# broadinstitute/colab-repeat-finder

Measured on AMD Instinct MI355X. Metric: Gbp/s scanned (motif 1-50), higher is better.
Workload: dtype u32 bit planes (2-bit bases)

## Files before the change

### colab-repeat-finder_amd/csrc/prf_plan.h

```cpp
#pragma once
#include <stdint.h>

typedef unsigned long long u64;
typedef unsigned int u32;

#define PRF_VMAX_K 480
#define PRF_VMAX_TASKS 80
#define PRF_VMAX_WAVES 4
#define PRF_GATHER_SLOTS_MAX 64u
#define PRF_GATHER_SUPER 64u
#define PRF_LAUNCH_MIXED 0x80000000u

struct alignas(4) prf_vtask {
    unsigned short k0;
    unsigned char kind;
    unsigned char valid;
    unsigned char stride;
    unsigned char pad;
    unsigned short item0;
};

struct prf_vplan {
    u32 n_waves;
    u32 n_tasks;
    u32 wave_begin[PRF_VMAX_WAVES + 1];
    prf_vtask tasks[PRF_VMAX_TASKS];
    u32 nc;
    u32 lds_bytes;
    u32 cof_words;
    u32 n_group_k;
    u32 n_exact;
    u32 k_exact0;
    u32 ticket_wave;
    u32 slack_waves;
    u32 per_cu;
    u32 prio;
};


namespace prf_layout {
constexpr int T = 32;
constexpr int RG = T / 4;
constexpr int LIN_PRE = 2;
constexpr int LIN_POST = 24;
constexpr int TILE_WORDS = 1024;
constexpr int LW = TILE_WORDS + LIN_PRE + LIN_POST;
constexpr int REC_CAP = 192;
constexpr int FLAG_CAP = 960;
constexpr int SLOW_CAP = 16;
constexpr int SMALL_M = 15;
constexpr int ROW_CAP_LDS = 448;
constexpr int SMEM_HDR = 240;
}

static inline long long prf_plan_min_matches(u32 k, u32 min_repeats, u32 min_span) {
    const long long a = (long long)(min_repeats - 1) * (long long)k, b = (long long)min_span - (long long)k;
    return a > b ? a : b;
}

bool prf_vertical_plan(u32 kmin, u32 kmax, u32 min_repeats, u32 min_span, prf_vplan *plan);
int prf_plan_json(u32 kmin, u32 kmax, u32 min_repeats, u32 min_span, char *buf, u64 buf_len);
```

### colab-repeat-finder_amd/csrc/scan_host.cpp

```cpp
#include <hip/hip_runtime.h>

#include <algorithm>
#include <chrono>
#include <cstdio>
#include <cstdlib>
#include <cstring>
#include <vector>

#include "genome.h"

template <class T>
static int grow(T *&p, u64 &cap, u64 want) {
    if (want <= cap) return PRF_OK;
    (void)hipFree(p);
    p = nullptr;
    cap = 0;
    HIPCHK(hipMalloc((void **)&p, want * sizeof(T)));
    cap = want;
    return PRF_OK;
}

static u64 with_headroom(u64 n) { return n + n / 8 + 1024; }

extern "C" {
// ... 91 lines not shown
    c->slab_slots = nslots;
    c->slab_cap = cap;
    return PRF_OK;
}

static int launch_fused(prf_ctx *c, const prf_genome *g, const prf_vplan &plan, const scan_params &p, prf_hit_dev *rows, u64 rows_cap,
                        u32 count_row, u64 *host_counters_dev, u64 *seq_out) {
    const launch_view lv = active_launch(g);
    prf_vscan_args a;
    a.VH = g->vp.VH; a.VL = g->vp.VL;
    a.H = g->H; a.L = g->L; a.X = g->X;
    a.E = g->d_E;
    a.launch_list = lv.list; a.n_launch = lv.n; a.flat_base = lv.flat;
    a.slabs = c->d_slabs; a.long_ends = c->d_long_ends; a.slab_count = c->d_slab_count; a.block_sum = c->d_block_sum; a.slab_cap = c->slab_cap;
    a.gather_shift = lv.n <= 8192u ? 3u : 5u;
#ifdef PRF_DIAG
    {
        static const int gs_env = getenv("PRF_GATHER_SHIFT") ? atoi(getenv("PRF_GATHER_SHIFT")) : -1;
        if (gs_env >= 3 && gs_env <= 6) a.gather_shift = (u32)gs_env;
    }
    {
        static const u32 skip_env = getenv("PRF_SKIP") ? (u32)strtoul(getenv("PRF_SKIP"), nullptr, 0) : 0u;
        a.skip = skip_env;
    }
#endif
    a.super_off = (lv.n + (1u << a.gather_shift) - 1u) >> a.gather_shift;
    a.min_repeats = p.min_repeats; a.min_span = p.min_span;
    a.tile_info = g->d_tile_info;
    a.counters = c->d_vcounters + (size_t)c->parity * PRF_CNT_N;
    a.dbg = nullptr;
#ifdef PRF_STAMPS
    {
        static u64 *dbg_buf = nullptr;
        const size_t nu = (size_t)(1u << 18) * PRF_VMAX_WAVES * 16;
        if (!dbg_buf) HIPCHK(hipMalloc((void **)&dbg_buf, nu * sizeof(u64)));
        if (lv.n <= (1u << 18)) {
            HIPCHK(hipMemsetAsync(dbg_buf, 0, (size_t)lv.n * PRF_VMAX_WAVES * 16 * sizeof(u64), c->stream));
            a.dbg = dbg_buf;
            c->stamps_buf = dbg_buf;
            c->stamps_n = lv.n;
        }
    }
#endif
    a.plan = plan;
    prf_vgather_args ga;
    ga.slabs = c->d_slabs; ga.long_ends = c->d_long_ends; ga.launch_list = lv.list; ga.flat_base = lv.flat; ga.tile_info = g->d_tile_info;
    ga.slab_count = c->d_slab_count; ga.block_sum = c->d_block_sum; ga.slab_cap = c->slab_cap; ga.n_launch = lv.n;
    ga.super_off = a.super_off;
    ga.gather_shift = a.gather_shift;
    ga.rows = rows; ga.rows_cap = rows_cap; ga.count_row = count_row;
    ga.counters = a.counters;
    ga.host_counters = host_counters_dev;
    ga.seq = ++c->scan_seq;
    ga.next_counters = c->d_vcounters + (size_t)(c->parity ^ 1u) * PRF_CNT_N;
    c->parity ^= 1u;
    const hipEvent_t *ev = ring_events(c, ga.seq);
    HIPCHK(hipEventRecord(ev[0], c->stream));
    hipError_t le = prf_vertical_launch(c->stream, a);
    if (le == hipSuccess) le = hipEventRecord(ev[1], c->stream);
    if (le == hipSuccess) le = prf_vertical_gather(c->stream, ga);
    if (le != hipSuccess) {
        reset_vcounters(c);
        return fail(PRF_EHIP, "fused scan launch failed: %s", hipGetErrorString(le));
    }
    HIPCHK(hipEventRecord(ev[2], c->stream));
    *seq_out = ga.seq;
    return PRF_OK;
}

struct row_dest {
// ... 35 lines not shown
    r.sorted = h[PRF_CNT_UNSORTED] == 0;
    r.ncand = shard_sum(h, PRF_SH_CAND);
    r.launches = 2;
    return r;
}

static void fill_stats(prf_scan_stats *s, const pass_result &r, u32 path, u64 positions, u32 tiles, u64 seq) {
    memset(s, 0, sizeof *s);
    s->phase1_ms = r.ms01;
    s->phase2_ms = r.ms12;
    s->scan_ms = (double)r.ms01 + (double)r.ms12;
    s->positions = positions;
    s->packed_bytes = (positions + 3) / 4;
    s->n_candidates = r.ncand;
    s->n_hits = r.nhits;
    s->n_launches = r.launches;
    s->path = path;
    s->seq = seq;
    s->sorted_on_device = r.sorted ? 1u : 0u;
    s->tiles_launched = tiles;
}

#ifdef PRF_STAMPS
static int dump_stamps(prf_ctx *c, const prf_vplan &plan) {
    const char *path = getenv("PRF_STAMPS_OUT");
    if (!path) return PRF_OK;
    fprintf(stderr, "[prf] plan: %u waves, %u tasks\n", plan.n_waves, plan.n_tasks);
    for (u32 w = 0; w < plan.n_waves; w++)
        for (u32 ti = plan.wave_begin[w]; ti < plan.wave_begin[w + 1]; ti++)
            fprintf(stderr, "[prf]   wave %u slot %u: kind %u k0 %u valid %02x stride %u\n", w, ti - plan.wave_begin[w],
                    plan.tasks[ti].kind, plan.tasks[ti].k0, plan.tasks[ti].valid, plan.tasks[ti].stride);
    if (c->stamps_buf) {
        HIPCHK(hipStreamSynchronize(c->stream));
        const size_t nu = (size_t)c->stamps_n * PRF_VMAX_WAVES * 16;
        std::vector<u64> host(nu);
        HIPCHK(hipMemcpy(host.data(), c->stamps_buf, nu * sizeof(u64), hipMemcpyDeviceToHost));
        if (FILE *f = fopen(path, "wb")) { fwrite(host.data(), 8, nu, f); fclose(f); }
    }
    return PRF_OK;
}
#endif

static int fused_pass(prf_ctx *c, const prf_genome *g, const prf_vplan &plan, const scan_params &p, const row_dest &dst, bool timed,
                      buffer_sizes *want, pass_result *r) {
    u64 seq = 0;
    int rc = launch_fused(c, g, plan, p, dst.rows, dst.cap, dst.is_sink ? 1u : 0u, c->h_counters_dev, &seq);
    if (rc) return rc;
    rc = wait_for_seq(c, seq);
    if (rc) return rc;
#ifdef PRF_STAMPS
    rc = dump_stamps(c, plan);
    if (rc) return rc;
#endif
    if (dst.is_sink) HIPCHK(hipStreamSynchronize(c->stream));
    const u64 *h = c->h_counters;
    *r = read_fused(h);
    if (timed) {
        const hipEvent_t *ev = ring_events(c, seq);
        HIPCHK(hipEventSynchronize(ev[2]));
        HIPCHK(hipEventElapsedTime(&r->ms01, ev[0], ev[2]));
    }
#ifdef PRF_DIAG
    if (getenv("PRF_DEBUG"))
        fprintf(stderr, "[prf] fused: hits %llu cand-records %llu (verified on the spot, a list being full: %llu) hit_ovf %llu unsorted %llu ms %.4f\n",
                (unsigned long long)r->nhits, (unsigned long long)r->ncand, (unsigned long long)shard_sum(h, PRF_SH_EARLY),
                (unsigned long long)h[PRF_CNT_HIT_OVF], (unsigned long long)h[PRF_CNT_UNSORTED], r->ms01);
#endif
// ... 275 lines not shown
```

### colab-repeat-finder_amd/csrc/scan_vertical.h

```cpp
#pragma once
#include <hip/hip_runtime.h>

#include <vector>

#include "prf_device.h"

#include "prf_plan.h"

struct prf_vplanes {
    u32 *VH = nullptr, *VL = nullptr;
    unsigned char *tile_class = nullptr;
    u32 *launch_list = nullptr;
    u32 n_launch = 0;
    u32 flat_base = ~0u;
    u64 ntiles_alloc = 0;
    std::vector<unsigned char> h_class;
    std::vector<u32> h_list;
};

#define PRF_LONG_PER_TILE 4u

struct prf_vscan_args {
    const u32 *VH, *VL;
    const u64 *H, *L, *X;
    const u64 *const *E;
    const u32 *launch_list;
    u32 n_launch;
    u32 flat_base;
    u64 *slabs;
    u64 *long_ends;
    u32 *slab_count;
    u32 *block_sum;
    u32 super_off;
    u32 gather_shift;
    u32 slab_cap;
    u32 min_repeats, min_span;
    const uint4 *tile_info;
    u64 *counters;
    u64 *dbg;
#ifdef PRF_DIAG
    u32 skip;
#endif
    prf_vplan plan;
};

struct prf_vgather_args {
    const u64 *slabs;
    const u64 *long_ends;
    const u32 *slab_count;
    const u32 *launch_list;
    u32 flat_base;
    const uint4 *tile_info;
    u32 *block_sum;
// ... 22 lines not shown
```

### colab-repeat-finder_amd/csrc/scan_vertical.hip

```cpp
#include <algorithm>
#include <cstdio>
#include <cstdlib>
#include <utility>
#include <vector>

#include "prf_host.h"
#include "prf_static_for.h"
#include "scan_vertical.h"
#include "verify_impl.h"

namespace {

#include "vscan_common.h"
#include "vscan_verify.h"
#include "vscan_tasks.h"

__device__ __forceinline__ void set_prio(u32 p) {
#ifdef PRF_NO_PRIO
    return;
#endif
    if (p == 0u) __builtin_amdgcn_s_setprio(0);
    else if (p == 1u) __builtin_amdgcn_s_setprio(1);
    else if (p == 2u) __builtin_amdgcn_s_setprio(2);
    else __builtin_amdgcn_s_setprio(3);
// ... 114 lines not shown
        tcw->slab_cap = g.slab_cap;
        tcw->min_repeats = g.min_repeats;
        tcw->min_span = g.min_span;
        tcw->lin_off = R1_OFF;
        tcw->keys_off = KEYS_OFF;
        tcw->slow_off = SLOW_OFF;
        tcw->k_exact0 = g.plan.k_exact0;
        tcw->cof_off = BITEMS_OFF + 4u * g.plan.n_group_k;
    }

    const u32 xcd = blockIdx.x & 7u;
    const u32 first_ticket = (gridDim.x - xcd + 7u) >> 3;
    u64 *ticket_word = g.counters + (PRF_CNT_SHARD0 + xcd * PRF_CNT_SHARD_STRIDE + PRF_SH_TILE_TICKET);
    prf_lds_u32 *next_words = (prf_lds_u32 *)(prf_smem + HDR_NEXT);
    u32 slot_next = 0;
    u32 parity = 0;
    prf_lds_u32 *wg_stats = (prf_lds_u32 *)(prf_smem + HDR_STATS);
    if (tid0 == 0) wg_stats[0] = wg_stats[1] = 0;
    for (u32 slot = blockIdx.x; slot < g.n_launch; slot = slot_next, parity ^= 1u) {
    int wave_s = wave;
    asm volatile("" : "+s"(wave_s));
    u32 ones = ~0u;
    asm volatile("" : "+s"(ones));
    int tid = wave_s * 64 + (int)__builtin_amdgcn_mbcnt_hi(ones, __builtin_amdgcn_mbcnt_lo(ones, 0u));
    asm volatile("" : "+v"(tid));
    const int lane = tid & 63;
    const u32 entry = sr.entry;
    const bool hasx = (entry & PRF_LAUNCH_MIXED) != 0;
    const u64 tile = entry & ~PRF_LAUNCH_MIXED;
    prf_lds_u32 *cnt = smem_cnt(parity);

    PRF_STAMP(0);
#ifdef PRF_STAMPS
    if (g.dbg && lane == 0) g.dbg[((u64)slot * MAX_WAVES + wave) * 16 + 12] = __builtin_amdgcn_s_memrealtime();
#endif
    set_prio(g.plan.prio & 3u);
    {
        sr.store(vimg, tid);
        if (hasx && tid < 64) {
            const u32 *px = reinterpret_cast<const u32 *>(g.X + tile * PRF_TILE_WORDS);
            u32 m = 0;
#pragma unroll 1
            for (u32 b0 = 0; b0 < 32u; b0 += 8u) {
                u32 v[8];
                static_for<0, 8>([&](auto bc) { v[decltype(bc)::value] = *(prf_glb_cu32 *)(px + ((b0 + (u32)decltype(bc)::value) * 64u + (u32)tid)); });
                static_for<0, 8>([&](auto bc) { m |= (v[decltype(bc)::value] == ~0u ? 1u : 0u) << (b0 + (u32)decltype(bc)::value); });
            }
            nostart[tid] = m;
        }
        if (tid < 8) cnt[tid] = 0;
        if (tid == 0) {
            TileCtx *tcw = reinterpret_cast<TileCtx *>(prf_smem);
            tcw->w0 = tile * PRF_TILE_WORDS - LIN_PRE;
            tcw->xz_lo = hasx ? 0 : tile * PRF_TILE;
            tcw->xz_hi = hasx ? 0 : (tile + 2) * PRF_TILE;
            tcw->slab = (prf_glb_u64 *)(g.slabs + (u64)slot * g.slab_cap);
            tcw->tile_base = tile * PRF_TILE;
            tcw->has_lin = 0u;
            tcw->cnt_off = (u32)HDR_CNT + 32u * parity;
        }
    }
    PRF_STAMP(1);
    __syncthreads();
    PRF_STAMP(2);

    set_prio(((g.plan.slack_waves >> wave) & 1u) ? (g.plan.prio >> 4) & 3u : (g.plan.prio >> 2) & 3u);
    Emit em;
    em.recs = recs;
    em.cnt = cnt;
    em.lane = lane;
#ifdef PRF_STAMPS
    u64 *task_dbg = g.dbg ? g.dbg + ((u64)slot * MAX_WAVES + wave) * 16 : nullptr;
#else
    u64 *task_dbg = nullptr;
#endif
    {
        u32 allow = hasx ? ~nostart[lane] : ~0u;
        if (vscan_skip(g) & 1u) allow = 0u;
        run_tasks<NC>((prf_lds_cu4 *)vimg, hotw, g.plan, wave, lane, hasx, allow, em, task_dbg);
    }
    constexpr u32 WIN_UNITS = (u32)LW;
    constexpr u32 WIN_PIECES = (WIN_UNITS + 63u) / 64u;
    static_assert(WIN_PIECES == 17, "the window's pieces are dealt 9 + 8 to the first two waves to arrive");
    prf_u32x4 wv[9];
    u32 order = 0;
    {
        if (lane == 0) order = atomicAdd((u32 *)(cnt + CNT_ROWS0), 1u);
        order = (u32)__builtin_amdgcn_readfirstlane((int)order);
        const long long w0 = (long long)(tile * PRF_TILE_WORDS) - LIN_PRE;
        const u64 *wh = g.H + w0, *wl = g.L + w0;
        const prf_u32x4 z = {0, 0, 0, 0};
        static_for<0, 9>([&](auto ic) { wv[decltype(ic)::value] = z; });
        if (order < 2u) {
            const u32 first = order * 9u, n = order ? 8u : 9u;
            static_for<0, 9>([&](auto ic) {
                constexpr u32 i = (u32)decltype(ic)::value;
                if (i < n) {
                    const u32 u = (first + i) * 64u + (u32)lane;
                    const u64 *src = u < (u32)LW / 2u ? wh + 2u * u : wl + 2u * (u - (u32)LW / 2u);
                    if (u < WIN_UNITS) wv[i] = *reinterpret_cast<const prf_u32x4 *>(src);
                }
            });
        }
    }
    u64 ticket = 0;
    const bool ticket_thread = order == 0u && lane == 0;
    if (ticket_thread) ticket = atomicAdd(ticket_word, 1ull);
    PRF_STAMP(3);
    __syncthreads();
    {
        if (order < 2u) {
            const u32 first = order * 9u, n = order ? 8u : 9u;
            static_for<0, 9>([&](auto ic) {
                constexpr u32 i = (u32)decltype(ic)::value;
                if (i < n) {
                    const u32 u = (first + i) * 64u + (u32)lane;
                    if (u < WIN_UNITS) *(prf_lds_u4 *)(prf_smem + R1_OFF + 16u * u) = wv[i];
                }
            });
        }
        const u32 n0 = cnt[CNT_ROWS];
        for (u32 i = (u32)tid; i < (u32)ROW_CAP_LDS; i += (u32)NTH)
            if (i >= n0) keys[i] = 0xFFFFFFFFu;
        if (tid == 0) {
            reinterpret_cast<TileCtx *>(prf_smem)->has_lin = 1u;
            cnt[CNT_ROWS0] = n0;
            cnt[CNT_LONG0] = cnt[CNT_LONG];
        }
    }
    u32 slot_pre = 0, entry_pre = entry;
    if (ticket_thread) {
        slot_pre = (first_ticket + (u32)ticket) * 8u + xcd;
        if (slot_pre < g.n_launch) entry_pre = entry_of(slot_pre);
    }
    __syncthreads();
    PRF_STAMP(4);

    set_prio(wave < MAX_WAVES / 2 ? (g.plan.prio >> 6) & 3u : (g.plan.prio >> 8) & 3u);
    const u32 *xw = hasx ? reinterpret_cast<const u32 *>(g.X + ((long long)(tile * PRF_TILE_WORDS) - LIN_PRE)) : nullptr;
    typedef const unsigned short __attribute__((address_space(3))) prf_lds_cu16;
    u32 n_recs = cnt[CNT_RECS], n_flags = cnt[CNT_FLAGS];
    {
        if (tid == 0) {
            const u32 early = cnt[CNT_EARLY];
            wg_stats[0] += n_flags + n_recs + early;
            wg_stats[1] += early;
        }
        n_recs = n_recs < (u32)REC_CAP ? n_recs : (u32)REC_CAP;
        n_flags = n_flags < (u32)FLAG_CAP ? n_flags : (u32)FLAG_CAP;
#ifdef PRF_STAMPS
        if (g.dbg && tid == 0) g.dbg[((u64)slot * MAX_WAVES + 0) * 16 + 11] = (u64)n_flags | ((u64)n_recs << 32);
#endif
        if (vscan_skip(g) & 2u) n_flags = 0;
        if (vscan_skip(g) & 4u) n_recs = 0;
        verify_all((prf_lds_cu64 *)recs, n_recs, (prf_lds_cu32 *)bitems, (vscan_skip(g) & 8u) ? 0u : g.plan.n_group_k, (prf_lds_cu16 *)hotw, n_flags, xw, (u32)tid, task_dbg);
    }
    set_prio((g.plan.prio >> 10) & 3u);
    if (ticket_thread) {
        next_words[0] = slot_pre;
        next_words[1] = entry_pre;
    }
    PRF_STAMP(5);
    __syncthreads();
    {
        const u32 n_slow = (u32)__builtin_amdgcn_readfirstlane((int)cnt[CNT_SLOW]);
        if (n_slow) {
            if (n_slow <= (u32)SLOW_CAP) {
                if ((u32)tid < n_slow) {
                    prf_lds_u64 *slow = (prf_lds_u64 *)(prf_smem + SLOW_OFF);
                    slow_item(slow[2u * (u32)tid], slow[2u * (u32)tid + 1u]);
                }
            } else {
                if (tid == 0) {
                    cnt[CNT_ROWS] = cnt[CNT_ROWS0];
                    cnt[CNT_LONG] = cnt[CNT_LONG0];
                }
                __syncthreads();
                verify_general((prf_lds_cu64 *)recs, n_recs, (prf_lds_cu32 *)bitems, g.plan.n_group_k, (prf_lds_cu16 *)hotw, n_flags, (u32)tid);
            }
            __syncthreads();
        }
    }
    PRF_STAMP(6);
    const u64 nw = *(prf_lds_u64 *)next_words;
    slot_next = (u32)__builtin_amdgcn_readfirstlane((int)(u32)nw);
    const u32 entry_next = (u32)(nw >> 32);
    const u32 n_rows = (vscan_skip(g) & 16u) ? 0u : (u32)__builtin_amdgcn_readfirstlane((int)cnt[CNT_ROWS]);
    const u32 n_long = (u32)__builtin_amdgcn_readfirstlane((int)cnt[CNT_LONG]);
    u64 *slab = g.slabs + (u64)slot * g.slab_cap;
    const u32 n_store = n_rows < g.slab_cap ? n_rows : g.slab_cap;
    bool unsorted = false;
    if (tid == 0) {
        g.slab_count[slot] = n_rows;
        if (n_store && !(vscan_skip(g) & 32u)) atomicAdd(&g.block_sum[slot >> g.gather_shift], n_store);
    }

    if (n_rows > (u32)ROW_CAP_LDS) {
        constexpr u32 R1_ROWS = R1_BYTES / 8u;
        static_assert(R1_ROWS % 32u == 0, "padding of the dense-tile key list");
        if (n_store <= R1_ROWS) {
            prf_lds_u32 *k2 = (prf_lds_u32 *)(prf_smem + R1_OFF), *v2 = k2 + R1_ROWS;
            for (u32 i = (u32)tid; i < (u32)ROW_CAP_LDS; i += (u32)NTH) {
                k2[i] = keys[i];
                v2[i] = keys[ROW_CAP_LDS + i];
            }
            for (u32 i = (u32)ROW_CAP_LDS + (u32)tid; i < n_store; i += (u32)NTH) {
                const u64 r = slab[i];
                k2[i] = (u32)r;
                v2[i] = (u32)(r >> 32);
            }
            for (u32 i = n_store + (u32)tid; i < ((n_store + 31u) & ~31u); i += (u32)NTH) k2[i] = 0xFFFFFFFFu;
            __syncthreads();
            typedef __attribute__((address_space(3))) const prf_u32x4 prf_lds_ckey4;
            prf_lds_ckey4 *k4 = (prf_lds_ckey4 *)k2;
            for (u32 r = (u32)tid; r < n_store; r += (u32)NTH) {
                const u32 mine = k2[r], kv = v2[r];
                u32 rank = 0;
                for (u32 c0 = 0; 4u * c0 < n_store; c0 += 8u) {
#pragma unroll
                    for (u32 j = 0; j < 8u; j++) {
                        const prf_u32x4 v = k4[c0 + j];
                        rank += (v.x < mine ? 1u : 0u) + (v.y < mine ? 1u : 0u) + (v.z < mine ? 1u : 0u) + (v.w < mine ? 1u : 0u);
                    }
                }
                slab[rank] = (u64)mine | ((u64)kv << 32);
            }
            __syncthreads();
        } else {
            for (u32 i = (u32)tid; i < (u32)ROW_CAP_LDS && i < n_store; i += (u32)NTH) slab[i] = (u64)keys[i] | ((u64)keys[ROW_CAP_LDS + i] << 32);
            unsorted = true;
        }
    }

    if (slot_next < g.n_launch) sr.load(g, entry_next, tid, wave, R1_OFF);
    else sr.clear();

    if (n_rows && n_rows <= (u32)ROW_CAP_LDS) {
        const u32 lg = n_rows > 128u ? 0u : (n_rows > 64u ? 1u : (n_rows > 32u ? 2u : 3u));
        const u32 P = 1u << lg, part = (u32)tid & (P - 1u);
        typedef __attribute__((address_space(3))) const prf_u32x4 prf_lds_ckey4;
        prf_lds_ckey4 *k4 = (prf_lds_ckey4 *)keys;
        for (u32 row0 = 0; row0 < n_rows; row0 += (u32)NTH >> lg) {
            const u32 row = row0 + ((u32)tid >> lg);
            const u32 r = row < n_rows ? row : 0u;
            const u32 mine = keys[r];
            const u32 kv = keys[ROW_CAP_LDS + r];
            u32 rank = 0;
            for (u32 c0 = part; 4u * c0 < n_rows; c0 += 8u * P) {
                prf_u32x4 v[8];
#pragma unroll
                for (u32 j = 0; j < 8u; j++) v[j] = k4[c0 + j * P];
                asm volatile("" : "+v"(v[0]), "+v"(v[1]), "+v"(v[2]), "+v"(v[3]), "+v"(v[4]), "+v"(v[5]), "+v"(v[6]), "+v"(v[7]));
#pragma unroll
                for (u32 j = 0; j < 8u; j++) {
                    rank += v[j].x < mine ? 1u : 0u;
                    rank += v[j].y < mine ? 1u : 0u;
                    rank += v[j].z < mine ? 1u : 0u;
                    rank += v[j].w < mine ? 1u : 0u;
                }
            }
            if (P >= 2u) rank += (u32)__builtin_amdgcn_update_dpp(0, (int)rank, 0xB1, 0xF, 0xF, true);
            if (P >= 4u) rank += (u32)__builtin_amdgcn_update_dpp(0, (int)rank, 0x4E, 0xF, 0xF, true);
            if (P >= 8u) rank += (u32)__builtin_amdgcn_update_dpp(0, (int)rank, 0x141, 0xF, 0xF, true);
            if (row < n_rows && part == 0 && rank < g.slab_cap && !(vscan_skip(g) & 64u)) slab[rank] = (u64)mine | ((u64)kv << 32);
        }
    }
    if ((u32)tid < n_long && (u32)tid < PRF_LONG_PER_TILE)
        g.long_ends[(u64)slot * PRF_LONG_PER_TILE + (u32)tid] = ((prf_lds_u64 *)(prf_smem + HDR_LONG))[tid];
    if (tid == 0) {
        if (n_rows > g.slab_cap) atomicMax(&g.counters[PRF_CNT_HIT_OVF], (u64)n_rows);
        if (unsorted) atomicMax(&g.counters[PRF_CNT_UNSORTED], 1ull);
        if (n_long > PRF_LONG_PER_TILE) atomicMax(&g.counters[PRF_CNT_LONG_OVF], (u64)n_long);
    }
    PRF_STAMP(7);
#ifdef PRF_STAMPS
    if (g.dbg && lane == 0) g.dbg[((u64)slot * MAX_WAVES + wave) * 16 + 13] = __builtin_amdgcn_s_memrealtime();
#endif
    }
    if (tid0 == 0) {
        const u64 cand_total = wg_stats[0], early_total = wg_stats[1];
        if (cand_total) atomicAdd(&g.counters[PRF_CNT_SHARD0 + (blockIdx.x % PRF_CNT_NSHARD) * PRF_CNT_SHARD_STRIDE + PRF_SH_CAND], cand_total);
        if (early_total) atomicAdd(&g.counters[PRF_CNT_SHARD0 + (blockIdx.x % PRF_CNT_NSHARD) * PRF_CNT_SHARD_STRIDE + PRF_SH_EARLY], early_total);
    }
}

}

static u32 resident_per_cu(u32 nc, u32 lds) {
    int n = 0;
    hipError_t e = nc == 72 ? hipOccupancyMaxActiveBlocksPerMultiprocessor(&n, prf_vscan_kernel<72>, NTH, lds)
                            : hipOccupancyMaxActiveBlocksPerMultiprocessor(&n, prf_vscan_kernel<80>, NTH, lds);
    if (e != hipSuccess || n < 1) {
        (void)hipGetLastError();
        n = (int)std::max(1u, (160u * 1024u) / std::max(1u, lds + 1280u));
    }
    return (u32)std::min(n, 6);
}

hipError_t prf_vertical_launch(hipStream_t s, const prf_vscan_args &args) {
    if (args.n_launch == 0) return hipSuccess;
    u32 lds = args.plan.lds_bytes;
#ifdef PRF_DIAG
    static const u32 lds_pad = getenv("PRF_LDS_PAD") ? (u32)atoi(getenv("PRF_LDS_PAD")) : 0u;
    lds += lds_pad;
#endif
    static int n_cu = 0;
    if (n_cu == 0) {
        int dev = 0;
        hipDeviceProp_t prop;
// ... 21 lines not shown
```

### colab-repeat-finder_amd/csrc/vscan_common.h

```cpp

using prf_layout::T; using prf_layout::RG; using prf_layout::LIN_PRE; using prf_layout::LIN_POST; using prf_layout::LW;
static_assert(prf_layout::TILE_WORDS == (int)PRF_TILE_WORDS, "tile size");
static_assert(LW % 2 == 0, "the window travels in 16-byte pieces");
constexpr u32 WIN_LEAD = 64u * (u32)LIN_PRE;
using prf_layout::REC_CAP; using prf_layout::FLAG_CAP; using prf_layout::SLOW_CAP;
constexpr int MAX_WAVES = PRF_VMAX_WAVES;
constexpr int NTH = 64 * MAX_WAVES;
using prf_layout::SMALL_M;
using prf_layout::ROW_CAP_LDS;
static_assert(ROW_CAP_LDS % 32 == 0, "the rank loop reads the padded key list 32 keys at a time");

__device__ __forceinline__ u64 make_rec(u32 lane, u32 k, u32 sc, u32 word) {
    return (u64)(lane | (k << 6) | (sc << 15)) | ((u64)word << 17);
}

typedef u32 prf_u32x2 __attribute__((ext_vector_type(2)));
typedef __attribute__((address_space(3))) prf_u32x2 prf_lds_u32x2;
static_assert(PRF_VMAX_K < (1 << 9), "k is a 9-bit field of a record");
__device__ __forceinline__ u32 make_rec_tag(u32 lane, u32 k, u32 sc) { return lane | (k << 6) | (sc << 15); }
__device__ __forceinline__ prf_u32x2 make_rec_halves(u32 tag, u32 word) {
    prf_u32x2 r = {tag | (word << 17), word >> 15};
    return r;
}

extern __shared__ __attribute__((aligned(16))) unsigned char prf_smem[];
using prf_layout::SMEM_HDR;
constexpr int HDR_CNT = 128;
constexpr int HDR_NEXT = 192;
constexpr int HDR_LONG = 200;
constexpr int HDR_STATS = 232;
static_assert(HDR_LONG + 8 * (int)PRF_LONG_PER_TILE <= HDR_STATS && HDR_STATS + 8 <= SMEM_HDR, "LDS header layout");
constexpr u32 CNT_ROWS = 0, CNT_RECS = 1, CNT_EARLY = 2, CNT_LONG = 3, CNT_FLAGS = 4, CNT_SLOW = 5,
              CNT_ROWS0 = 6, CNT_LONG0 = 7;

typedef u32 prf_u32x4 __attribute__((ext_vector_type(4)));
typedef __attribute__((address_space(3))) const prf_u32x4 prf_lds_cu4;
typedef __attribute__((address_space(3))) prf_u32x4 prf_lds_u4;
typedef __attribute__((address_space(3))) u64 prf_lds_u64;
typedef __attribute__((address_space(3))) u32 prf_lds_u32;
typedef __attribute__((address_space(3))) const u32 prf_lds_cu32;
typedef __attribute__((address_space(3))) void prf_lds_void;
typedef __attribute__((address_space(1))) const void prf_glb_cvoid;
typedef __attribute__((address_space(1))) const u32 prf_glb_cu32;
typedef __attribute__((address_space(1))) u64 prf_glb_u64;

#ifdef PRF_STAMPS
#define PRF_STAMP(i)                                                                                               \
    do {                                                                                                           \
        if (g.dbg && lane == 0) g.dbg[((u64)slot * MAX_WAVES + wave) * 16 + (i)] = __builtin_amdgcn_s_memtime(); \
    } while (0)
#else
#define PRF_STAMP(i) do { } while (0)
#endif

struct TileCtx {
    u64 w0;
    u64 xz_lo, xz_hi;
    const u64 *H, *L, *X;
    const u64 *const *E;
    prf_glb_u64 *slab;
    u64 tile_base;
    u32 slab_cap;
    u32 min_repeats, min_span;
    u32 lin_off;
    u32 has_lin;
    u32 keys_off;
    u32 cof_off;
    u32 slow_off;
    u32 k_exact0;
    u32 cnt_off;
};
static_assert(sizeof(TileCtx) <= 128, "TileCtx must fit its LDS header slot");

struct CofTable {
    u32 v[PRF_VMAX_K + 4];
    constexpr CofTable() : v{} {
        for (u32 k = 2; k <= PRF_VMAX_K; k++) {
            u32 rest = k, packed = 0, n = 0;
            for (u32 p = 2; p <= rest; p++) {
                if (rest % p) continue;
                packed |= (k / p) << (8 * n++);
                while (rest % p == 0) rest /= p;
            }
            v[k] = packed;
        }
// ... 4 lines not shown
```

### colab-repeat-finder_amd/csrc/vscan_verify.h

```cpp

__device__ __forceinline__ void emit_row(const TileCtx &tc, u64 a, u64 b, u32 k) {
    const u64 span = b + k - a;
    prf_lds_u32 *cnt = (prf_lds_u32 *)(prf_smem + tc.cnt_off);
    u32 kv = k;
    if (span >= 65535ull) {
        const u32 j = atomicAdd((u32 *)(cnt + CNT_LONG), 1u);
        if (j < PRF_LONG_PER_TILE) {
            ((prf_lds_u64 *)(prf_smem + HDR_LONG))[j] = b + k;
            kv |= (j + 1u) << 16;
        }
    }
    const u32 key = ((u32)(a - tc.tile_base) << 16) | (span < 65535ull ? (u32)span : 65535u);
    const u32 i = atomicAdd((u32 *)(cnt + CNT_ROWS), 1u);
    if (i < (u32)ROW_CAP_LDS) {
        prf_lds_u32 *keys = (prf_lds_u32 *)(prf_smem + tc.keys_off);
        keys[i] = key;
        keys[ROW_CAP_LDS + i] = kv;
    } else if (i < tc.slab_cap) {
        tc.slab[i] = (u64)key | ((u64)kv << 32);
    }
}

__device__ __noinline__ u64 tile_mismatch64(u64 q, u32 k) {
    const TileCtx &tc = *reinterpret_cast<const TileCtx *>(prf_smem);
    prf_window_view view;
    view.lds = (prf_lds_cu64 *)(prf_smem + tc.lin_off);
    view.w0 = tc.w0;
    view.nwords = tc.has_lin ? LW : 0;
    view.xz_lo = tc.xz_lo;
    view.xz_hi = tc.xz_hi;
    view.x_in_lds = 0;
    view.P[0] = tc.H; view.P[1] = tc.L; view.P[2] = tc.X;
    view.E = tc.E;
    return view.mismatch64(q, k);
}

__device__ __forceinline__ u64 run_end(u64 from, u32 k) {
    u64 b = from;
    for (;;) {
        const u64 m2 = tile_mismatch64(b, k);
        if (m2) return b + (u64)__builtin_ctzll(m2);
        b += 64;
    }
}

__device__ __forceinline__ bool motif_is_repeat(u64 a, u32 k) {
    const TileCtx &tc = *reinterpret_cast<const TileCtx *>(prf_smem);
    for (u32 cf = ((prf_lds_cu32 *)(prf_smem + tc.cof_off))[k]; cf; cf >>= 8) {
        const u32 d = cf & 255u, need = k - d;
        bool has = true;
        for (u32 off = 0; off < need; off += 64) {
            u64 mm = tile_mismatch64(a + off, d);
// ... 313 lines not shown
    const u32 c = lo ? (u32)__builtin_clz(lo) : 32u;
    if (c == 0 || c >= back) return;
    const u64 a = tile_end - c;
    const u64 hi = mm >> 32;
    u64 b;
    if (hi) {
        b = tile_end + (u64)__builtin_ctzll(hi);
    } else {
        u32 from = WIN_LEAD + PRF_TILE + 32u;
        if (!win_run_end(wc, from, k, b)) {
            defer(tc, a, k, 0u, 0u, 1u, wc.win0 + from);
            return;
        }
    }
    if (b - a < (u64)min_matches32(k, tc.min_repeats, tc.min_span)) return;
    static_assert(WIN_LEAD + PRF_TILE + 2u * PRF_VMAX_K + 96u <= WIN_POS, "the motif of a boundary item lies inside the window");
    if (!win_motif_is_repeat(wc, WIN_LEAD + PRF_TILE - c, k)) emit_row(tc, a, b, k);
}

__device__ __forceinline__ void boundary_general(const TileCtx &tc, u32 k, u32 S) {
    const u64 tile_end = tc.tile_base + PRF_TILE;
    const u32 back = 8u * S;
    const u64 mm = tile_mismatch64(tile_end - 32, k);
    const u32 lo = (u32)mm;
    const u32 c = lo ? (u32)__builtin_clz(lo) : 32u;
    if (c == 0 || c >= back) return;
    const u64 a = tile_end - c;
    const u64 hi = mm >> 32;
    const u64 b = hi ? tile_end + (u64)__builtin_ctzll(hi) : run_end(tile_end + 32, k);
    if (b - a < (u64)min_matches32(k, tc.min_repeats, tc.min_span)) return;
    if (!motif_is_repeat(a, k)) emit_row(tc, a, b, k);
}

__device__ __forceinline__ prf_lds_u32 *smem_cnt(u32 parity) { return (prf_lds_u32 *)(prf_smem + HDR_CNT) + 8u * parity; }

__device__ __forceinline__ void verify_all(prf_lds_cu64 *recs, u32 n_recs, prf_lds_cu32 *bitems, u32 n_bitems, const unsigned short __attribute__((address_space(3))) *flags,
                                           u32 n_flags, const u32 *xw, u32 tid, u64 *dbg) {
#ifdef PRF_STAMPS
#define PRF_VSTAMP(i) do { if (dbg && (tid & 63u) == 0) dbg[i] = __builtin_amdgcn_s_memtime(); } while (0)
#else
#define PRF_VSTAMP(i) do { } while (0)
#endif
    const TileCtx &tc = *reinterpret_cast<const TileCtx *>(prf_smem);
    WinCtx wc;
    wc.h = (prf_lds_cu32 *)(prf_smem + tc.lin_off);
    wc.l = wc.h + 2 * LW;
    wc.xw = xw;
    wc.cof = (prf_lds_cu32 *)(prf_smem + tc.cof_off);
    wc.win0 = tc.tile_base - WIN_LEAD;
    wc.min_repeats = tc.min_repeats;
    wc.min_span = tc.min_span;
    if (tid >= (u32)NTH / 2u) {
        const u32 up = (u32)NTH - 1u - tid;
        const u32 hwl = tid & 63u;
        prf_lds_u32 *list = (prf_lds_u32 *)(prf_smem + LEAD_OFF) + (up >> 6) * LEAD_CAP;
        u32 idx = 2u * (up & 63u) + (up >> 6), word = 0, head = 0;
        for (;;) {
            u32 n_items = 0;
            bool more;
            for (;;) {
                if (word == 0u && idx < n_recs) {
                    const u64 rec = recs[idx];
                    idx += (u32)NTH / 2u;
                    head = (u32)rec & 0x1FFFFu;
                    word = (u32)(rec >> 17);
                }
                const u32 pc = (u32)__builtin_popcount(word);
// ... 92 lines not shown
```

Before: 6182.

## Bucket emitted rows into four key-range sublists ranked per wave

Emitted rows now go into one of four LDS sublists chosen by the top two key bits, each with its own counter, and rows past a sublist's capacity go to a separate overflow slab region. The per-tile rank sort then has each wave rank only its own sublist and add an offset, using alignbit/popcount comparisons instead of every thread scanning the full key list. The dense path merges sublists and overflow into a bucketed order before ranking within each bucket. This cuts the quadratic rank work and the LDS traffic, at the cost of more header counters, more complex overflow handling, and possible load imbalance when keys cluster in one quarter.

```diff
diff --git a/colab-repeat-finder_amd/csrc/prf_plan.h b/colab-repeat-finder_amd/csrc/prf_plan.h
--- a/colab-repeat-finder_amd/csrc/prf_plan.h
+++ b/colab-repeat-finder_amd/csrc/prf_plan.h
@@ -49,8 +49,9 @@
 constexpr int FLAG_CAP = 960;
 constexpr int SLOW_CAP = 16;
 constexpr int SMALL_M = 15;
-constexpr int ROW_CAP_LDS = 448;
-constexpr int SMEM_HDR = 240;
+constexpr int QCAP = 112;
+constexpr int ROW_CAP_LDS = 4 * QCAP;
+constexpr int SMEM_HDR = 304;
 }
 
 static inline long long prf_plan_min_matches(u32 k, u32 min_repeats, u32 min_span) {
diff --git a/colab-repeat-finder_amd/csrc/scan_host.cpp b/colab-repeat-finder_amd/csrc/scan_host.cpp
--- a/colab-repeat-finder_amd/csrc/scan_host.cpp
+++ b/colab-repeat-finder_amd/csrc/scan_host.cpp
@@ -147,10 +147,10 @@
 #ifdef PRF_STAMPS
     {
         static u64 *dbg_buf = nullptr;
-        const size_t nu = (size_t)(1u << 18) * PRF_VMAX_WAVES * 16;
+        const size_t nu = (size_t)(1u << 18) * PRF_VMAX_WAVES * PRF_STAMP_SLOTS;
         if (!dbg_buf) HIPCHK(hipMalloc((void **)&dbg_buf, nu * sizeof(u64)));
         if (lv.n <= (1u << 18)) {
-            HIPCHK(hipMemsetAsync(dbg_buf, 0, (size_t)lv.n * PRF_VMAX_WAVES * 16 * sizeof(u64), c->stream));
+            HIPCHK(hipMemsetAsync(dbg_buf, 0, (size_t)lv.n * PRF_VMAX_WAVES * PRF_STAMP_SLOTS * sizeof(u64), c->stream));
             a.dbg = dbg_buf;
             c->stamps_buf = dbg_buf;
             c->stamps_n = lv.n;
@@ -252,7 +252,7 @@
                     plan.tasks[ti].kind, plan.tasks[ti].k0, plan.tasks[ti].valid, plan.tasks[ti].stride);
     if (c->stamps_buf) {
         HIPCHK(hipStreamSynchronize(c->stream));
-        const size_t nu = (size_t)c->stamps_n * PRF_VMAX_WAVES * 16;
+        const size_t nu = (size_t)c->stamps_n * PRF_VMAX_WAVES * PRF_STAMP_SLOTS;
         std::vector<u64> host(nu);
         HIPCHK(hipMemcpy(host.data(), c->stamps_buf, nu * sizeof(u64), hipMemcpyDeviceToHost));
         if (FILE *f = fopen(path, "wb")) { fwrite(host.data(), 8, nu, f); fclose(f); }
diff --git a/colab-repeat-finder_amd/csrc/scan_vertical.h b/colab-repeat-finder_amd/csrc/scan_vertical.h
--- a/colab-repeat-finder_amd/csrc/scan_vertical.h
+++ b/colab-repeat-finder_amd/csrc/scan_vertical.h
@@ -19,6 +19,7 @@
 };
 
 #define PRF_LONG_PER_TILE 4u
+#define PRF_STAMP_SLOTS 24
 
 struct prf_vscan_args {
     const u32 *VH, *VL;
diff --git a/colab-repeat-finder_amd/csrc/scan_vertical.hip b/colab-repeat-finder_amd/csrc/scan_vertical.hip
--- a/colab-repeat-finder_amd/csrc/scan_vertical.hip
+++ b/colab-repeat-finder_amd/csrc/scan_vertical.hip
@@ -170,7 +170,7 @@
 
     PRF_STAMP(0);
 #ifdef PRF_STAMPS
-    if (g.dbg && lane == 0) g.dbg[((u64)slot * MAX_WAVES + wave) * 16 + 12] = __builtin_amdgcn_s_memrealtime();
+    if (g.dbg && lane == 0) g.dbg[((u64)slot * MAX_WAVES + wave) * PRF_STAMP_SLOTS + 12] = __builtin_amdgcn_s_memrealtime();
 #endif
     set_prio(g.plan.prio & 3u);
     {
@@ -186,7 +186,7 @@
             }
             nostart[tid] = m;
         }
-        if (tid < 8) cnt[tid] = 0;
+        if (tid < (int)CNT_N) cnt[tid] = 0;
         if (tid == 0) {
             TileCtx *tcw = reinterpret_cast<TileCtx *>(prf_smem);
             tcw->w0 = tile * PRF_TILE_WORDS - LIN_PRE;
@@ -195,7 +195,7 @@
             tcw->slab = (prf_glb_u64 *)(g.slabs + (u64)slot * g.slab_cap);
             tcw->tile_base = tile * PRF_TILE;
             tcw->has_lin = 0u;
-            tcw->cnt_off = (u32)HDR_CNT + 32u * parity;
+            tcw->cnt_off = (u32)HDR_CNT + 4u * CNT_N * parity;
         }
     }
     PRF_STAMP(1);
@@ -208,7 +208,7 @@
     em.cnt = cnt;
     em.lane = lane;
 #ifdef PRF_STAMPS
-    u64 *task_dbg = g.dbg ? g.dbg + ((u64)slot * MAX_WAVES + wave) * 16 : nullptr;
+    u64 *task_dbg = g.dbg ? g.dbg + ((u64)slot * MAX_WAVES + wave) * PRF_STAMP_SLOTS : nullptr;
 #else
     u64 *task_dbg = nullptr;
 #endif
@@ -257,12 +257,19 @@
                 }
             });
         }
-        const u32 n0 = cnt[CNT_ROWS];
-        for (u32 i = (u32)tid; i < (u32)ROW_CAP_LDS; i += (u32)NTH)
-            if (i >= n0) keys[i] = 0xFFFFFFFFu;
+        const prf_u32x4 n0 = *(prf_lds_cu4 *)(cnt + CNT_ROWS);
+        for (u32 i = (u32)tid; i < (u32)ROW_CAP_LDS; i += (u32)NTH) {
+            const u32 q = i / (u32)QCAP, j = i - q * (u32)QCAP;
+            const u32 n0q = q == 0u ? n0.x : (q == 1u ? n0.y : (q == 2u ? n0.z : n0.w));
+            if (j >= n0q) keys[i] = quarter_pad(q);
+        }
         if (tid == 0) {
             reinterpret_cast<TileCtx *>(prf_smem)->has_lin = 1u;
-            cnt[CNT_ROWS0] = n0;
+            cnt[CNT_ROWS0] = n0.x;
+            cnt[CNT_ROWS0 + 1u] = n0.y;
+            cnt[CNT_ROWS0 + 2u] = n0.z;
+            cnt[CNT_ROWS0 + 3u] = n0.w;
+            cnt[CNT_OVF0] = cnt[CNT_OVF];
             cnt[CNT_LONG0] = cnt[CNT_LONG];
         }
     }
@@ -287,7 +294,7 @@
         n_recs = n_recs < (u32)REC_CAP ? n_recs : (u32)REC_CAP;
         n_flags = n_flags < (u32)FLAG_CAP ? n_flags : (u32)FLAG_CAP;
 #ifdef PRF_STAMPS
-        if (g.dbg && tid == 0) g.dbg[((u64)slot * MAX_WAVES + 0) * 16 + 11] = (u64)n_flags | ((u64)n_recs << 32);
+        if (g.dbg && tid == 0) g.dbg[((u64)slot * MAX_WAVES + 0) * PRF_STAMP_SLOTS + 11] = (u64)n_flags | ((u64)n_recs << 32);
 #endif
         if (vscan_skip(g) & 2u) n_flags = 0;
         if (vscan_skip(g) & 4u) n_recs = 0;
@@ -310,7 +317,8 @@
                 }
             } else {
                 if (tid == 0) {
-                    cnt[CNT_ROWS] = cnt[CNT_ROWS0];
+                    for (u32 q = 0; q < 4u; q++) cnt[CNT_ROWS + q] = cnt[CNT_ROWS0 + q];
+                    cnt[CNT_OVF] = cnt[CNT_OVF0];
                     cnt[CNT_LONG] = cnt[CNT_LONG0];
                 }
                 __syncthreads();
@@ -323,7 +331,17 @@
     const u64 nw = *(prf_lds_u64 *)next_words;
     slot_next = (u32)__builtin_amdgcn_readfirstlane((int)(u32)nw);
     const u32 entry_next = (u32)(nw >> 32);
-    const u32 n_rows = (vscan_skip(g) & 16u) ? 0u : (u32)__builtin_amdgcn_readfirstlane((int)cnt[CNT_ROWS]);
+    u32 nq0, nq1, nq2, nq3;
+    {
+        const prf_u32x4 c = *(prf_lds_cu4 *)(cnt + CNT_ROWS);
+        const bool none = (vscan_skip(g) & 16u) != 0;
+        nq0 = none ? 0u : (u32)__builtin_amdgcn_readfirstlane((int)c.x);
+        nq1 = none ? 0u : (u32)__builtin_amdgcn_readfirstlane((int)c.y);
+        nq2 = none ? 0u : (u32)__builtin_amdgcn_readfirstlane((int)c.z);
+        nq3 = none ? 0u : (u32)__builtin_amdgcn_readfirstlane((int)c.w);
+    }
+    const u32 n_rows = nq0 + nq1 + nq2 + nq3;
+    const bool dense = nq0 > (u32)QCAP || nq1 > (u32)QCAP || nq2 > (u32)QCAP || nq3 > (u32)QCAP;
     const u32 n_long = (u32)__builtin_amdgcn_readfirstlane((int)cnt[CNT_LONG]);
     u64 *slab = g.slabs + (u64)slot * g.slab_cap;
     const u32 n_store = n_rows < g.slab_cap ? n_rows : g.slab_cap;
@@ -333,39 +351,57 @@
         if (n_store && !(vscan_skip(g) & 32u)) atomicAdd(&g.block_sum[slot >> g.gather_shift], n_store);
     }
 
-    if (n_rows > (u32)ROW_CAP_LDS) {
+    if (dense) {
         constexpr u32 R1_ROWS = R1_BYTES / 8u;
-        static_assert(R1_ROWS % 32u == 0, "padding of the dense-tile key list");
-        if (n_store <= R1_ROWS) {
+        const u32 m0 = nq0 < (u32)QCAP ? nq0 : (u32)QCAP, m1 = nq1 < (u32)QCAP ? nq1 : (u32)QCAP, m2 = nq2 < (u32)QCAP ? nq2 : (u32)QCAP,
+                  m3 = nq3 < (u32)QCAP ? nq3 : (u32)QCAP;
+        const u32 n_ovf = n_rows - (m0 + m1 + m2 + m3);
+        const u32 s1 = nq0, s2 = nq0 + nq1, s3 = s2 + nq2;
+        auto pick = [](u32 q, u32 a0, u32 a1, u32 a2, u32 a3) -> u32 { return q == 0u ? a0 : (q == 1u ? a1 : (q == 2u ? a2 : a3)); };
+        if (n_rows <= g.slab_cap && n_rows <= R1_ROWS) {
             prf_lds_u32 *k2 = (prf_lds_u32 *)(prf_smem + R1_OFF), *v2 = k2 + R1_ROWS;
+            prf_lds_u32 *fill = cnt + CNT_ROWS0;
+            if (tid < 4) fill[tid] = pick((u32)tid, m0, m1, m2, m3);
             for (u32 i = (u32)tid; i < (u32)ROW_CAP_LDS; i += (u32)NTH) {
-                k2[i] = keys[i];
-                v2[i] = keys[ROW_CAP_LDS + i];
-            }
-            for (u32 i = (u32)ROW_CAP_LDS + (u32)tid; i < n_store; i += (u32)NTH) {
+                const u32 q = i / (u32)QCAP, j = i - q * (u32)QCAP;
+                if (j < pick(q, m0, m1, m2, m3)) {
+                    const u32 at = pick(q, 0u, s1, s2, s3) + j;
+                    k2[at] = keys[i];
+                    v2[at] = keys[ROW_CAP_LDS + i];
+                }
+            }
+            __syncthreads();
+            for (u32 i = (u32)tid; i < n_ovf; i += (u32)NTH) {
                 const u64 r = slab[i];
-                k2[i] = (u32)r;
-                v2[i] = (u32)(r >> 32);
-            }
-            for (u32 i = n_store + (u32)tid; i < ((n_store + 31u) & ~31u); i += (u32)NTH) k2[i] = 0xFFFFFFFFu;
+                const u32 q = (u32)r >> 30;
+                const u32 at = pick(q, 0u, s1, s2, s3) + atomicAdd((u32 *)(fill + q), 1u);
+                k2[at] = (u32)r;
+                v2[at] = (u32)(r >> 32);
+            }
+            for (u32 i = n_rows + (u32)tid; i < ((n_rows + 3u) & ~3u); i += (u32)NTH) k2[i] = 0xFFFFFFFFu;
             __syncthreads();
             typedef __attribute__((address_space(3))) const prf_u32x4 prf_lds_ckey4;
             prf_lds_ckey4 *k4 = (prf_lds_ckey4 *)k2;
-            for (u32 r = (u32)tid; r < n_store; r += (u32)NTH) {
+            for (u32 r = (u32)tid; r < n_rows; r += (u32)NTH) {
                 const u32 mine = k2[r], kv = v2[r];
-                u32 rank = 0;
-                for (u32 c0 = 0; 4u * c0 < n_store; c0 += 8u) {
-#pragma unroll
-                    for (u32 j = 0; j < 8u; j++) {
-                        const prf_u32x4 v = k4[c0 + j];
-                        rank += (v.x < mine ? 1u : 0u) + (v.y < mine ? 1u : 0u) + (v.z < mine ? 1u : 0u) + (v.w < mine ? 1u : 0u);
-                    }
+                const u32 q = mine >> 30;
+                const u32 lo = pick(q, 0u, s1, s2, s3), hi = lo + pick(q, nq0, nq1, nq2, nq3);
+                const u32 u_lo = lo >> 2, u_hi = (hi + 3u) >> 2;
+                u32 rank = 4u * u_lo;
+#pragma unroll 4
+                for (u32 u = u_lo; u < u_hi; u++) {
+                    const prf_u32x4 v = k4[u];
+                    rank += (v.x < mine ? 1u : 0u) + (v.y < mine ? 1u : 0u) + (v.z < mine ? 1u : 0u) + (v.w < mine ? 1u : 0u);
                 }
                 slab[rank] = (u64)mine | ((u64)kv << 32);
             }
             __syncthreads();
         } else {
-            for (u32 i = (u32)tid; i < (u32)ROW_CAP_LDS && i < n_store; i += (u32)NTH) slab[i] = (u64)keys[i] | ((u64)keys[ROW_CAP_LDS + i] << 32);
+            for (u32 i = (u32)tid; i < (u32)ROW_CAP_LDS; i += (u32)NTH) {
+                const u32 q = i / (u32)QCAP, j = i - q * (u32)QCAP;
+                const u32 at = n_ovf + pick(q, 0u, m0, m0 + m1, m0 + m1 + m2) + j;
+                if (j < pick(q, m0, m1, m2, m3) && at < g.slab_cap) slab[at] = (u64)keys[i] | ((u64)keys[ROW_CAP_LDS + i] << 32);
+            }
             unsorted = true;
         }
     }
@@ -373,34 +409,50 @@
     if (slot_next < g.n_launch) sr.load(g, entry_next, tid, wave, R1_OFF);
     else sr.clear();
 
-    if (n_rows && n_rows <= (u32)ROW_CAP_LDS) {
-        const u32 lg = n_rows > 128u ? 0u : (n_rows > 64u ? 1u : (n_rows > 32u ? 2u : 3u));
-        const u32 P = 1u << lg, part = (u32)tid & (P - 1u);
-        typedef __attribute__((address_space(3))) const prf_u32x4 prf_lds_ckey4;
-        prf_lds_ckey4 *k4 = (prf_lds_ckey4 *)keys;
-        for (u32 row0 = 0; row0 < n_rows; row0 += (u32)NTH >> lg) {
-            const u32 row = row0 + ((u32)tid >> lg);
-            const u32 r = row < n_rows ? row : 0u;
-            const u32 mine = keys[r];
-            const u32 kv = keys[ROW_CAP_LDS + r];
-            u32 rank = 0;
-            for (u32 c0 = part; 4u * c0 < n_rows; c0 += 8u * P) {
-                prf_u32x4 v[8];
-#pragma unroll
-                for (u32 j = 0; j < 8u; j++) v[j] = k4[c0 + j * P];
-                asm volatile("" : "+v"(v[0]), "+v"(v[1]), "+v"(v[2]), "+v"(v[3]), "+v"(v[4]), "+v"(v[5]), "+v"(v[6]), "+v"(v[7]));
-#pragma unroll
-                for (u32 j = 0; j < 8u; j++) {
-                    rank += v[j].x < mine ? 1u : 0u;
-                    rank += v[j].y < mine ? 1u : 0u;
-                    rank += v[j].z < mine ? 1u : 0u;
-                    rank += v[j].w < mine ? 1u : 0u;
-                }
-            }
-            if (P >= 2u) rank += (u32)__builtin_amdgcn_update_dpp(0, (int)rank, 0xB1, 0xF, 0xF, true);
-            if (P >= 4u) rank += (u32)__builtin_amdgcn_update_dpp(0, (int)rank, 0x4E, 0xF, 0xF, true);
-            if (P >= 8u) rank += (u32)__builtin_amdgcn_update_dpp(0, (int)rank, 0x141, 0xF, 0xF, true);
-            if (row < n_rows && part == 0 && rank < g.slab_cap && !(vscan_skip(g) & 64u)) slab[rank] = (u64)mine | ((u64)kv << 32);
+    PRF_RANK_DECL();
+    {
+        const u32 nq = wave_s == 0 ? nq0 : (wave_s == 1 ? nq1 : (wave_s == 2 ? nq2 : nq3));
+        const u32 below = wave_s == 0 ? 0u : (wave_s == 1 ? nq0 : (wave_s == 2 ? nq0 + nq1 : nq0 + nq1 + nq2));
+        if (nq && !dense) {
+            const u32 lg = nq > 32u ? 0u : (nq > 16u ? 1u : 2u);
+            const u32 P = 1u << lg, part = (u32)lane & (P - 1u);
+            const u32 units = (nq + 3u) >> 2;
+            prf_lds_u32 *sub = keys + (u32)wave_s * (u32)QCAP;
+            typedef __attribute__((address_space(3))) const prf_u32x4 prf_lds_ckey4;
+            prf_lds_ckey4 *k4 = (prf_lds_ckey4 *)sub + part;
+            for (u32 row0 = 0; row0 < nq; row0 += 64u >> lg) {
+                const u32 row = row0 + ((u32)lane >> lg);
+                const u32 r = row < nq ? row : 0u;
+                PRF_RANK_T0();
+                const u32 mine = sub[r];
+                const u32 kv = sub[ROW_CAP_LDS + r];
+                u32 rank = 0;
+                auto batch = [&](u32 u0, auto nc) {
+                    constexpr u32 N = (u32)decltype(nc)::value;
+                    prf_u32x4 v[N];
+                    static_for<0, (int)N>([&](auto jc) { v[decltype(jc)::value] = k4[u0 + (u32)decltype(jc)::value * P]; });
+                    if constexpr (N == 4u) asm volatile("" : "+v"(v[0]), "+v"(v[1]), "+v"(v[2]), "+v"(v[3]));
+                    else asm volatile("" : "+v"(v[0]), "+v"(v[1]));
+                    u32 bits = 0;
+                    static_for<0, (int)N>([&](auto jc) {
+                        constexpr u32 j = (u32)decltype(jc)::value;
+                        bits = __builtin_amdgcn_alignbit(bits, v[j].x - mine, 31);
+                        bits = __builtin_amdgcn_alignbit(bits, v[j].y - mine, 31);
+                        bits = __builtin_amdgcn_alignbit(bits, v[j].z - mine, 31);
+                        bits = __builtin_amdgcn_alignbit(bits, v[j].w - mine, 31);
+                    });
+                    rank += (u32)__builtin_popcount(bits);
+                };
+                for (u32 u0 = 0; u0 < units; u0 += 4u * P) {
+                    if (units - u0 > 2u * P) batch(u0, std::integral_constant<u32, 4>{});
+                    else batch(u0, std::integral_constant<u32, 2>{});
+                }
+                if (P >= 2u) rank += (u32)__builtin_amdgcn_update_dpp(0, (int)rank, 0xB1, 0xF, 0xF, true);
+                if (P >= 4u) rank += (u32)__builtin_amdgcn_update_dpp(0, (int)rank, 0x4E, 0xF, 0xF, true);
+                PRF_RANK_T1(rank);
+                rank += below;
+                if (row < nq && part == 0 && rank < g.slab_cap && !(vscan_skip(g) & 64u)) slab[rank] = (u64)mine | ((u64)kv << 32);
+            }
         }
     }
     if ((u32)tid < n_long && (u32)tid < PRF_LONG_PER_TILE)
@@ -411,8 +463,9 @@
         if (n_long > PRF_LONG_PER_TILE) atomicMax(&g.counters[PRF_CNT_LONG_OVF], (u64)n_long);
     }
     PRF_STAMP(7);
+    PRF_RANK_STORE();
 #ifdef PRF_STAMPS
-    if (g.dbg && lane == 0) g.dbg[((u64)slot * MAX_WAVES + wave) * 16 + 13] = __builtin_amdgcn_s_memrealtime();
+    if (g.dbg && lane == 0) g.dbg[((u64)slot * MAX_WAVES + wave) * PRF_STAMP_SLOTS + 13] = __builtin_amdgcn_s_memrealtime();
 #endif
     }
     if (tid0 == 0) {
diff --git a/colab-repeat-finder_amd/csrc/vscan_common.h b/colab-repeat-finder_amd/csrc/vscan_common.h
--- a/colab-repeat-finder_amd/csrc/vscan_common.h
+++ b/colab-repeat-finder_amd/csrc/vscan_common.h
@@ -7,8 +7,8 @@
 constexpr int MAX_WAVES = PRF_VMAX_WAVES;
 constexpr int NTH = 64 * MAX_WAVES;
 using prf_layout::SMALL_M;
-using prf_layout::ROW_CAP_LDS;
-static_assert(ROW_CAP_LDS % 32 == 0, "the rank loop reads the padded key list 32 keys at a time");
+using prf_layout::ROW_CAP_LDS; using prf_layout::QCAP;
+static_assert(QCAP % 16 == 0 && ROW_CAP_LDS == 4 * QCAP, "a wave ranks one sublist in 16-byte reads, batches of up to four per lane, that stay inside it");
 
 __device__ __forceinline__ u64 make_rec(u32 lane, u32 k, u32 sc, u32 word) {
     return (u64)(lane | (k << 6) | (sc << 15)) | ((u64)word << 17);
@@ -26,12 +26,14 @@
 extern __shared__ __attribute__((aligned(16))) unsigned char prf_smem[];
 using prf_layout::SMEM_HDR;
 constexpr int HDR_CNT = 128;
-constexpr int HDR_NEXT = 192;
-constexpr int HDR_LONG = 200;
-constexpr int HDR_STATS = 232;
+constexpr int HDR_NEXT = 256;
+constexpr int HDR_LONG = 264;
+constexpr int HDR_STATS = 296;
 static_assert(HDR_LONG + 8 * (int)PRF_LONG_PER_TILE <= HDR_STATS && HDR_STATS + 8 <= SMEM_HDR, "LDS header layout");
-constexpr u32 CNT_ROWS = 0, CNT_RECS = 1, CNT_EARLY = 2, CNT_LONG = 3, CNT_FLAGS = 4, CNT_SLOW = 5,
-              CNT_ROWS0 = 6, CNT_LONG0 = 7;
+constexpr u32 CNT_N = 16, CNT_ROWS = 0, CNT_RECS = 4, CNT_EARLY = 5, CNT_LONG = 6, CNT_FLAGS = 7, CNT_SLOW = 8, CNT_OVF = 9,
+              CNT_ROWS0 = 10, CNT_OVF0 = 14, CNT_LONG0 = 15;
+static_assert(HDR_CNT % 16 == 0 && CNT_ROWS % 4 == 0 && HDR_CNT + 2 * 4 * (int)CNT_N <= HDR_NEXT, "the four row counters are one 16-byte read");
+__device__ __forceinline__ u32 quarter_pad(u32 q) { return ((q + 1u) << 30) - 1u; }
 
 typedef u32 prf_u32x4 __attribute__((ext_vector_type(4)));
 typedef __attribute__((address_space(3))) const prf_u32x4 prf_lds_cu4;
@@ -47,10 +49,25 @@
 #ifdef PRF_STAMPS
 #define PRF_STAMP(i)                                                                                               \
     do {                                                                                                           \
-        if (g.dbg && lane == 0) g.dbg[((u64)slot * MAX_WAVES + wave) * 16 + (i)] = __builtin_amdgcn_s_memtime(); \
+        if (g.dbg && lane == 0) g.dbg[((u64)slot * MAX_WAVES + wave) * PRF_STAMP_SLOTS + (i)] = __builtin_amdgcn_s_memtime(); \
+    } while (0)
+#define PRF_RANK_DECL() u64 rank_cyc = 0, rank_t0 = 0
+#define PRF_RANK_T0() do { rank_t0 = __builtin_amdgcn_s_memtime(); } while (0)
+#define PRF_RANK_T1(v)                                            \
+    do {                                                          \
+        asm volatile("" : "+v"(v));                               \
+        rank_cyc += __builtin_amdgcn_s_memtime() - rank_t0;       \
+    } while (0)
+#define PRF_RANK_STORE()                                                                                    \
+    do {                                                                                                    \
+        if (g.dbg && lane == 0) g.dbg[((u64)slot * MAX_WAVES + wave) * PRF_STAMP_SLOTS + 16] = rank_cyc; \
     } while (0)
 #else
 #define PRF_STAMP(i) do { } while (0)
+#define PRF_RANK_DECL() do { } while (0)
+#define PRF_RANK_T0() do { } while (0)
+#define PRF_RANK_T1(v) do { } while (0)
+#define PRF_RANK_STORE() do { } while (0)
 #endif
 
 struct TileCtx {
diff --git a/colab-repeat-finder_amd/csrc/vscan_verify.h b/colab-repeat-finder_amd/csrc/vscan_verify.h
--- a/colab-repeat-finder_amd/csrc/vscan_verify.h
+++ b/colab-repeat-finder_amd/csrc/vscan_verify.h
@@ -11,13 +11,15 @@
         }
     }
     const u32 key = ((u32)(a - tc.tile_base) << 16) | (span < 65535ull ? (u32)span : 65535u);
-    const u32 i = atomicAdd((u32 *)(cnt + CNT_ROWS), 1u);
-    if (i < (u32)ROW_CAP_LDS) {
-        prf_lds_u32 *keys = (prf_lds_u32 *)(prf_smem + tc.keys_off);
+    const u32 q = key >> 30;
+    const u32 i = atomicAdd((u32 *)(cnt + CNT_ROWS + q), 1u);
+    if (i < (u32)QCAP) {
+        prf_lds_u32 *keys = (prf_lds_u32 *)(prf_smem + tc.keys_off) + q * (u32)QCAP;
         keys[i] = key;
         keys[ROW_CAP_LDS + i] = kv;
-    } else if (i < tc.slab_cap) {
-        tc.slab[i] = (u64)key | ((u64)kv << 32);
+    } else {
+        const u32 j = atomicAdd((u32 *)(cnt + CNT_OVF), 1u);
+        if (j < tc.slab_cap) tc.slab[j] = (u64)key | ((u64)kv << 32);
     }
 }
 
@@ -397,7 +399,7 @@
     if (!motif_is_repeat(a, k)) emit_row(tc, a, b, k);
 }
 
-__device__ __forceinline__ prf_lds_u32 *smem_cnt(u32 parity) { return (prf_lds_u32 *)(prf_smem + HDR_CNT) + 8u * parity; }
+__device__ __forceinline__ prf_lds_u32 *smem_cnt(u32 parity) { return (prf_lds_u32 *)(prf_smem + HDR_CNT) + CNT_N * parity; }
 
 __device__ __forceinline__ void verify_all(prf_lds_cu64 *recs, u32 n_recs, prf_lds_cu32 *bitems, u32 n_bitems, const unsigned short __attribute__((address_space(3))) *flags,
                                            u32 n_flags, const u32 *xw, u32 tid, u64 *dbg) {
```

Result: faster. 6366, median of 6 (+3.0%).
